# zprodev/zlib.es

Measured on AMD Instinct MI355X. Metric: GiB/s deflate+inflate round trip, 64 MiB buffers (uncompressed bytes / wall), bit-exact vs reference, higher is better.
Workload: dtype u8; 1 GPU; random64: 1 x 64 MiB xorshift buffer(s) per GPU (seed 12345+index), deflate then inflate, HBM-resident; bytes_per_buffer=67108864, compressed_bytes=67176156, parallelism=independent buffers, one per GPU

## Files before the change

### zlib.es_amd/csrc/zes_api.hip

```cpp
#include "../../include/zes.h"
#include "zes_kernels.h"
#include "zes_chain.h"

#include <algorithm>
#include <atomic>
#include <condition_variable>
#include <cstdio>
#include <cstddef>
#include <cstdlib>
#include <cstring>
#include <chrono>
#include <functional>
#include <future>
#include <initializer_list>
#include <deque>
#include <map>
#include <mutex>
#include <string>
#include <thread>
#include <vector>

extern "C" int zes_gen(uint8_t* out, uint64_t n, uint32_t kind, uint32_t seed);

namespace {
// ... 587 lines not shown

hipEvent_t take_event() {
  if (!g.event_pool.empty()) {
    hipEvent_t e = g.event_pool.back();
    g.event_pool.pop_back();
    return e;
  }
  hipEvent_t e = nullptr;
  (void)hipEventCreate(&e);
  return e;
}

struct Timed {
  hipEvent_t a = nullptr, b = nullptr;
  const char* name;
  hipStream_t st;
  explicit Timed(const char* n, hipStream_t stream = nullptr) : name(n), st(stream ? stream : g.stream) {
    if (g.profiling) {
      a = take_event();
      b = take_event();
      (void)hipEventRecord(a, st);
    }
  }
  ~Timed() {
    if (g.profiling) {
      (void)hipEventRecord(b, st);
      g.pending.push_back({name, {a, b}});
    }
    static const bool trace = getenv("ZES_TRACE_KERNELS") != nullptr;
    if (trace) {
      const hipError_t e = hipStreamSynchronize(g.stream);
      fprintf(stderr, "zes kernel done: %s (%s)\n", name, hipGetErrorName(e));
      fflush(stderr);
    }
  }
};

void collect_times() {
  if (!g.profiling) return;
  std::map<std::string, KTime> acc;
  std::vector<std::string> order;
  for (auto& p : g.pending) {
    float ms = 0;
    (void)hipEventSynchronize(p.second.second);
    (void)hipEventElapsedTime(&ms, p.second.first, p.second.second);
    if (!acc.count(p.first)) order.push_back(p.first);
    acc[p.first].ms += ms;
    acc[p.first].launches++;
    g.event_pool.push_back(p.second.first);
    g.event_pool.push_back(p.second.second);
  }
  g.pending.clear();
  g.last_times.clear();
  for (auto& e : g.carry) {
    auto it = acc.find(e.first);
    if (it != acc.end()) {
      e.second.ms += it->second.ms;
      e.second.launches += it->second.launches;
      acc.erase(it);
    }
    g.last_times.push_back(e);
  }
  g.carry.clear();
  for (auto& n : order)
    if (acc.count(n)) g.last_times.push_back({n, acc[n]});
}

void keep_times() {
  if (g.profiling) g.carry = g.last_times;
}

bool deflate_throws(uint64_t n) { return n == 0 || n == 1 || (n % ZES_BLK) == 1; }
uint64_t deflate_bound(uint64_t n) { return ((n < ZES_BLK / 2) ? (uint64_t)ZES_BLK : n * 2) + 6; }

using PhaseSetter = void (*)(unsigned long long*);
int phases_arm(PhaseSetter set, uint32_t nblk) {
  int rc = ensure(g.dbg, (size_t)nblk * 64);
  if (rc) return rc;
  HIPCHK(hipMemsetAsync(g.dbg.p, 0, (size_t)nblk * 64, g.stream));
  HIPCHK(hipStreamSynchronize(g.stream));
  set((unsigned long long*)g.dbg.p);
  return ZES_OK;
}
int phases_print(PhaseSetter set, uint32_t nblk, int ran, const char* fmt) {
  HIPCHK(hipStreamSynchronize(g.stream));
  set(nullptr);
  std::vector<unsigned long long> h((size_t)nblk * 8);
  HIPCHK(hipMemcpy(h.data(), g.dbg.p, h.size() * 8, hipMemcpyDeviceToHost));
  double acc[8] = {0};
  uint32_t n = 0;
  for (uint32_t i = 0; i < nblk; i++) {
    const unsigned long long* s = &h[(size_t)i * 8];
    if (!s[ran]) continue;
    n++;
    for (int k = 1; k < 8; k++) acc[k] += (double)(k <= ran ? s[k] - s[k - 1] : s[k]);
  }
  if (n) fprintf(stderr, fmt, n, acc[1] / n, acc[2] / n, acc[3] / n, acc[4] / n, acc[5] / n, acc[6] / n, acc[7] / n);
  return ZES_OK;
}

template <class F>
int launch_lz77(const uint8_t* d_in, uint32_t grid, bool use_index, bool heaviest_first, bool phases, F after_index, uint32_t* route = nullptr) {
  int rc;
  const ZesBuf* dbufs = (const ZesBuf*)g.bufs.p;
  ZesBlk* dblks = (ZesBlk*)g.blks.p;
  uint32_t* idx_a = (uint32_t*)g.idx_a.p;
  uint32_t* idx_b = (uint32_t*)g.idx_b.p;
  {
    Timed t("k_lz_sort");
    hipLaunchKernelGGL(k_lz_sort, dim3(grid), dim3(SORT_THREADS), 0, g.stream, d_in, dbufs, dblks, idx_a, idx_b, idx_a, (uint16_t*)g.sdelta.p,
                       ZES_SORT_MODE_FIRST | (use_index ? ZES_SORT_USE_INDEX : 0u));
  }
  auto note = [&](uint32_t* flag_to, uint32_t* word_to) -> int {
    HIPCHK(hipMemcpyAsync(flag_to, idx_a + ZES_BLK - 1, 4, hipMemcpyDeviceToHost, g.stream));
    if (word_to) HIPCHK(hipMemcpyAsync(word_to, idx_b + ZES_BLK - 1, 4, hipMemcpyDeviceToHost, g.stream));
    return ZES_OK;
  };
  if (route && (rc = note(&route[0], &route[3]))) return rc;
  if (use_index) {
    {
      Timed t("k_lz_index");
      hipLaunchKernelGGL(k_lz_index, dim3(grid), dim3(IDX_THREADS), 0, g.stream, d_in, dbufs, dblks, idx_a, idx_b, idx_a, (uint16_t*)g.sdelta.p);
    }
    if (route && (rc = note(&route[1], &route[4]))) return rc;
    {
      Timed t("k_lz_sort_redo");
      hipLaunchKernelGGL(k_lz_sort, dim3(grid), dim3(SORT_THREADS), 0, g.stream, d_in, dbufs, dblks, idx_a, idx_b, idx_a, (uint16_t*)g.sdelta.p,
                         ZES_SORT_MODE_REDO);
    }
    if (route && (rc = note(&route[2], nullptr))) return rc;
  }
  if ((rc = after_index())) return rc;
  {
    Timed t("k_lz_match");
    hipLaunchKernelGGL(k_lz_match, dim3(grid), dim3(MATCH_THREADS), 0, g.stream, d_in, dbufs, dblks, idx_a, idx_b, (uint32_t*)g.mlist.p);
  }
  if (phases && (rc = phases_arm(zes_lazy_set_dbg, grid))) return rc;
  {
    const uint32_t* order = nullptr;
    if (heaviest_first) {
      if ((rc = ensure(g.order, (size_t)grid * 4))) return rc;
      Timed t("k_lz_order");
      hipLaunchKernelGGL(k_lz_order, dim3(1), dim3(1024), 0, g.stream, (const uint32_t*)idx_a, grid, (uint32_t*)g.order.p);
      order = (const uint32_t*)g.order.p;
    }
    Timed t("k_lz_match_lazy");
    hipLaunchKernelGGL(k_lz_match_lazy, dim3(grid), dim3(MATCH_THREADS), 0, g.stream, d_in, dbufs, dblks, idx_a, (const uint32_t*)idx_a,
                       (const uint16_t*)g.sdelta.p, idx_b, (uint32_t*)g.tmask.p, (uint32_t*)g.mlist.p, order);
  }
  if (phases) {
    if ((rc = phases_print(zes_lazy_set_dbg, grid, 5,
                           "zes lazy match steps (avg cycles over %u blocks): stage %.0f tail %.0f window chains %.0f entry chains %.0f true chain (only unmerged blocks) %.0f | first wave, window chains: %.0f loop turns\n")))
      return rc;
    if ((rc = phases_arm(zes_parse_set_dbg, grid))) return rc;
  }
  {
    Timed t("k_lz_parse_small");
    hipLaunchKernelGGL(k_lz_parse_small, dim3(grid), dim3(PARSE_THREADS), 0, g.stream, d_in, dbufs, dblks, idx_b, idx_a, (uint32_t*)g.hists.p,
                       (const uint32_t*)g.tmask.p, (const uint32_t*)g.mlist.p);
  }
  {
    Timed t("k_lz_parse");
    hipLaunchKernelGGL(k_lz_parse, dim3(grid), dim3(PARSE_THREADS), 0, g.stream, d_in, dbufs, dblks, idx_b, idx_a, (uint32_t*)g.hists.p,
                       (const uint32_t*)g.tmask.p, (const uint32_t*)g.mlist.p);
  }
  return ZES_OK;
}

struct DeflateRange {
  uint64_t n_read = 0;
  uint32_t flags = 0;
  uint32_t start_bit = 0;
  bool defer = false;
  uint32_t adler = 1;
};

// ... 8 lines not shown
    out_len[i] = 0;
    if (deflate_throws(in_len[i])) {
      status[i] = ZES_E_CORRUPT;
      continue;
    }
    if (out_cap[i] < deflate_bound(in_len[i])) {
      status[i] = ZES_E_NOSPACE;
      out_len[i] = deflate_bound(in_len[i]);
      continue;
    }
    if ((out_off[i] & 15u) || (((uintptr_t)d_out) & 15u)) {
      status[i] = ZES_E_ARG;
      continue;
    }
    status[i] = ZES_OK;
    ZesBuf b;
    b.in_off = in_off[i];
    b.n = in_len[i];
    b.out_off = out_off[i];
    b.cap = out_cap[i];
    b.first_blk = (uint32_t)nblk_total;
    b.nblk = (uint32_t)((in_len[i] + ZES_BLK - 1) / ZES_BLK);
    b.n_read = one ? std::max(one->n_read, in_len[i]) : in_len[i];
    b.flags = one ? one->flags : 0u;
    b.start_bit = one ? one->start_bit : 0u;
    nblk_total += b.nblk;
    hb.push_back(b);
    live.push_back(i);
  }
  if (hb.empty()) return ZES_OK;
  if (nblk_total >= (1ull << 31)) return ZES_E_ARG;
  const uint32_t nbuf = (uint32_t)hb.size(), nblk = (uint32_t)nblk_total;
  int rc;
  if ((rc = ensure(g.bufs, sizeof(ZesBuf) * nbuf))) return rc;
  if ((rc = ensure(g.blks, sizeof(ZesBlk) * nblk))) return rc;
  if ((rc = ensure(g.idx_a, (size_t)nblk * ZES_BLK * 4))) return rc;
  if ((rc = ensure(g.idx_b, (size_t)nblk * ZES_BLK * 4))) return rc;
  if ((rc = ensure(g.sdelta, (size_t)nblk * ZES_BLK * 2 + 64))) return rc;
  if ((rc = ensure(g.tmask, (size_t)nblk * ZES_TMASK_WORDS * 4))) return rc;
  if ((rc = ensure(g.mlist, (size_t)nblk * ZES_MLIST_WORDS * 4))) return rc;
  if ((rc = ensure(g.hists, (size_t)nblk * 320 * 4))) return rc;
  if ((rc = ensure(g.codes, (size_t)nblk * 320 * 4))) return rc;
  if ((rc = ensure(g.hdrs, (size_t)nblk * ZES_HDR_WORDS * 4))) return rc;
  if ((rc = ensure(g.adler, (size_t)nbuf * 16))) return rc;
  if ((rc = ensure(g.res, sizeof(ZesRes) * nbuf))) return rc;
  ZesBuf* dbufs = (ZesBuf*)g.bufs.p;
  ZesBlk* dblks = (ZesBlk*)g.blks.p;
  unsigned long long* adler = (unsigned long long*)g.adler.p;
  if (nbuf > 1) {
    if (nbuf <= DEFLATE_TABLE_BUFS) {
      memcpy(g.pinned->def.table, hb.data(), sizeof(ZesBuf) * nbuf);
      HIPCHK(hipMemcpyAsync(g.bufs.p, g.pinned->def.table, sizeof(ZesBuf) * nbuf, hipMemcpyHostToDevice, g.stream));
    } else {
      HIPCHK(hipMemcpy(g.bufs.p, hb.data(), sizeof(ZesBuf) * nbuf, hipMemcpyHostToDevice));
    }
  }
  {
    Timed t("k_make_blks");
    const uint32_t nthr = std::max(nblk, 2u * nbuf);
    hipLaunchKernelGGL(k_make_blks, dim3((nthr + 255) / 256), dim3(256), 0, g.stream, hb[0], nbuf, dbufs, dblks, nblk, adler);
  }
  {
    HIPCHK(hipEventRecord(g.ev_a0, g.stream));
    HIPCHK(hipStreamWaitEvent(g.s_adler, g.ev_a0, 0));
    Timed t("k_adler", g.s_adler);
    if (nbuf == 1) {
      const uint32_t nch = (uint32_t)((hb[0].n + ADLER_CHUNK - 1) / ADLER_CHUNK);
      hipLaunchKernelGGL(k_adler, dim3(nch), dim3(ADLER_THREADS), 0, g.s_adler, d_in, hb[0].in_off, hb[0].n, adler);
    } else {
      hipLaunchKernelGGL(k_adler_blocks, dim3(nblk), dim3(ADLER_THREADS), 0, g.s_adler, d_in, dbufs, dblks, adler);
    }
  }
  HIPCHK(hipEventRecord(g.ev_a1, g.s_adler));
  const bool sort_dbg = getenv("ZES_DEBUG_PHASES") != nullptr;
  if (sort_dbg && (rc = phases_arm(zes_sort_set_dbg, nblk))) return rc;
  static const bool use_index = getenv("ZES_NO_INDEX") == nullptr;
  rc = launch_lz77(d_in, nblk, use_index, nbuf > 1 && nblk > 256, sort_dbg, [&]() -> int {
    if (!sort_dbg) return ZES_OK;
    return phases_print(zes_sort_set_dbg, nblk, 7,
                        "zes sort steps (avg cycles over %u blocks): zero %.0f count %.0f flags %.0f level 2 + compact %.0f stage %.0f three passes %.0f sd/inv %.0f\n");
  });
  if (rc) return rc;
  if (sort_dbg) {
    if ((rc = phases_print(zes_parse_set_dbg, nblk, 7, "zes parse steps (avg cycles over %u blocks): A %.0f B %.0f C %.0f D1 %.0f D2 %.0f D3 %.0f out %.0f\n"))) return rc;
    if ((rc = phases_arm(zes_huff_set_dbg, nblk))) return rc;
  }
  ZesRes* res_direct = (nbuf <= DEFLATE_DIRECT_BUFS && g.pinned_dev) ? g.pinned_dev->def.res : nullptr;
  {
    Timed t("k_huff");
    hipLaunchKernelGGL(k_huff, dim3(nblk), dim3(HUFF_THREADS_HOST), 0, g.stream, dblks, (const uint32_t*)g.hists.p,
                       (uint32_t*)g.codes.p, (uint32_t*)g.hdrs.p);
  }
  if (sort_dbg && (rc = phases_print(zes_huff_set_dbg, nblk, 7,
                                     "zes huff steps (avg cycles over %u blocks): rank sorts %.0f both alphabets' levels %.0f codes %.0f run-length coding %.0f its code %.0f header bits %.0f totals+out %.0f\n")))
    return rc;
  {
    HIPCHK(hipStreamWaitEvent(g.stream, g.ev_a1, 0));
    Timed t("k_layout");
    hipLaunchKernelGGL(k_layout, dim3(nbuf), dim3(256), 0, g.stream, d_out, dbufs, dblks, adler, res_direct ? res_direct : (ZesRes*)g.res.p);
  }
  if (sort_dbg && (rc = phases_arm(zes_emit_set_dbg, nblk))) return rc;
  {
    Timed t("k_emit");
    hipLaunchKernelGGL(k_emit, dim3(nblk), dim3(EMIT_THREADS), 0, g.stream, d_out, dbufs, dblks, (uint32_t*)g.idx_a.p,
                       (const uint32_t*)g.codes.p, (const uint32_t*)g.hdrs.p);
  }
  if (sort_dbg && (rc = phases_print(zes_emit_set_dbg, nblk, 1,
                                     "zes emit steps (avg cycles over %u blocks, first wave): whole %.0f = header copy %.0f build %.0f scan %.0f stage %.0f flush %.0f\n")))
    return rc;
  HIPCHK(hipGetLastError());
  ZesRes* r = g.pinned->def.res;
  if (nbuf > DEFLATE_DIRECT_BUFS) {
    if (nbuf > g.res_more_n) {
      if (g.res_more) HIPCHK(hipHostFree(g.res_more));
      g.res_more = nullptr;
      g.res_more_n = 0;
      HIPCHK(hipHostMalloc((void**)&g.res_more, sizeof(ZesRes) * nbuf * 2, hipHostMallocDefault));
      g.res_more_n = (size_t)nbuf * 2;
    }
    r = g.res_more;
  }
  if (!res_direct) HIPCHK(hipMemcpyAsync(r, g.res.p, sizeof(ZesRes) * nbuf, hipMemcpyDeviceToHost, g.stream));
  if (one && one->defer) return ZES_OK;
  HIPCHK(hipStreamSynchronize(g.stream));
  collect_times();
  for (uint32_t k = 0; k < nbuf; k++) {
    out_len[live[k]] = r[k].out_len;
    status[live[k]] = r[k].status;
  }
  if (one) one->adler = r[0].aux;
  return ZES_OK;
}

int deflate_one(const uint8_t* d_in, uint64_t in_off, uint64_t n, uint8_t* d_out, uint64_t out_off, uint64_t cap, uint64_t* out_len,
                DeflateRange* range = nullptr) {
  int32_t st = 0;
  const int rc = deflate_batch_core(d_in, &in_off, &n, d_out, &out_off, &cap, out_len, &st, 1, range);
  return rc ? rc : st;
}

int read_res(ZesRes* out) {
  HIPCHK(hipMemcpyAsync(&g.pinned->res1, g.res.p, sizeof(ZesRes), hipMemcpyDeviceToHost, g.stream));
  HIPCHK(hipStreamSynchronize(g.stream));
  *out = g.pinned->res1;
  return ZES_OK;
}

struct InfJob {
  uint64_t in_off, c, out_off, cap;
  uint64_t out_len;
  int status;
  int tier;
  uint32_t start0 = 16, hist = 0;
  bool partial = false, final_seen = false;
  uint64_t end_bit = 0;
  int btype0 = -1;
  bool want_end = false;
};

ZesInfBuf inf_buf(const InfJob& j) {
  ZesInfBuf b;
  memset(&b, 0, sizeof b);
  b.in_off = j.in_off;
  b.c = j.c;
  b.out_off = j.out_off;
  b.cap = j.cap;
  return b;
// ... 4913 lines not shown
```

### zlib.es_amd/csrc/zes_deflate.hip

```cpp
#include "zes_common.h"
#include "zes_kernels.h"

__device__ static inline uint32_t lds_ld32u(const uint8_t* s, uint32_t off) {
  const uint32_t* w = reinterpret_cast<const uint32_t*>(s);
  uint32_t i = off >> 2;
  uint32_t lo = w[i], hi = w[i + 1];
  return __builtin_amdgcn_alignbyte(hi, lo, off & 3u);
}

__device__ static inline void stage_block(uint8_t* s, const uint8_t* g, uint32_t bytes, uint32_t padded) {
  const uint32_t tid = threadIdx.x, nth = blockDim.x;
  const uint32_t mis = (uint32_t)((uintptr_t)g & 15u);
  if (mis == 0) {
    const uint4* g4 = reinterpret_cast<const uint4*>(g);
    uint4* s4 = reinterpret_cast<uint4*>(s);
    const uint32_t full = bytes >> 4;
    for (uint32_t i = tid; i < full; i += nth) s4[i] = g4[i];
    for (uint32_t i = (full << 4) + tid; i < padded; i += nth) s[i] = i < bytes ? g[i] : (uint8_t)0;
  } else {
    for (uint32_t i = tid; i < padded; i += nth) s[i] = i < bytes ? g[i] : (uint8_t)0;
  }
}

__device__ unsigned long long* g_sort_dbg = nullptr;
// ... 1646 lines not shown
              mo[base + lane] = LAZY_EVAL_LIT;
              atomicOr(&S.v1[(base + lane) >> 5], 1u << ((base + lane) & 31u));
            }
            p += nrun;
            continue;
          }
          if (++nev > budget3) {
            if (lane == 0) S.abort3 = 1u;
            break;
          }
          const uint32_t iv = (uint32_t)__builtin_amdgcn_readlane((int)ciw, (int)po);
          m = lazy_wave_eval(S, iv, sd, p, T, avail);
          if (lane == 0) mo[p] = m;
          if ((m & ZES_TOK_MATCH) && zes_tok_len(m) == ZES_MAXMATCH) {
            const uint32_t pj = p + ZES_MAXMATCH * (lane + 1u);
            const bool inr = pj < tbase && pj + ZES_MAXMATCH + 3u <= T && pj + ZES_MAXMATCH <= avail;
            const uint32_t ivj = inv[inr ? pj : 0u];
            const bool has = inr && ivj != ZES_INV_NONE;
            const uint32_t dj = sd[has ? (ivj & 0x1FFFFu) : 0u];
            const uint32_t qj = has ? pj - dj : 0u, pp = has ? pj : 0u;
            bool full = has;
            for (uint32_t wv = 0; wv < 32u && __ballot(full); wv += 4u) {
              uint64_t x = 0;
#pragma unroll
              for (uint32_t t = 0; t < 4u; t++) x |= lz_ld64(S.in, qj + 8u * (wv + t)) ^ lz_ld64(S.in, pp + 8u * (wv + t));
              full = full && x == 0ull;
            }
            full = full && ((lz_ld32(S.in, qj + 256u) ^ lz_ld32(S.in, pp + 256u)) & 0xffffu) == 0u;
            const uint64_t okm = __ballot(full);
            const uint32_t nk = (~okm) ? (uint32_t)__builtin_ctzll(~okm) : 64u;
            if (lane < nk) {
              mo[pj] = ZES_TOK_MATCH | ((ZES_MAXMATCH - 3u) << 16) | (dj - 1u);
              atomicOr(&S.v1[pj >> 5], 1u << (pj & 31u));
            }
            p += ZES_MAXMATCH * nk;
          }
        }
      }
      p += (m & ZES_TOK_MATCH) ? zes_tok_len(m) : 1u;
    }
    if (lane < 2u && cnt + lane < T && cnt + lane >= p) atomicOr(&S.v1[(cnt + lane) >> 5], 1u << ((cnt + lane) & 31u));
  }
  if (walk3) {
    __syncthreads();
    if (S.abort3) {
      probe = false;
      if (tid == 0) S.route |= ZES_ROUTE_ABORT3;
      __syncthreads();
      continue;
    }
    for (uint32_t i = tid; i < ZES_BLK / 32; i += MATCH_THREADS) tm[4u + i] = S.v1[i];
    __syncthreads();
    if (tid == 0) tm[0] = 1u;
  }
  break;
  }
  if (tid == 0) tm[1] = S.route;
  LSTAMP(5);
}

__device__ unsigned long long* g_parse_dbg = nullptr;
void zes_parse_set_dbg(unsigned long long* p) { (void)hipMemcpyToSymbol(HIP_SYMBOL(g_parse_dbg), &p, sizeof p); }
#define PSTAMP(i)                                                                                          \
  do {                                                                                                     \
    if (g_parse_dbg && threadIdx.x == 0) g_parse_dbg[(size_t)blockIdx.x * 8 + (i)] = (unsigned long long)clock64(); \
  } while (0)
#define PARSE_CHUNKS (ZES_BLK / 64)
#define PARSE_REGION 128
#define PARSE_NOENTRY 0xFFu
#define PARSE_BATCH 8u
template <bool SMALL>
struct ParseSmemT;
template <>
struct ParseSmemT<false> {
  union {
    uint8_t xmap[PARSE_CHUNKS][64];
    struct {
      unsigned long long mask[PARSE_CHUNKS];
      uint32_t cpre[PARSE_CHUNKS];
    } d;
  } u;
  uint16_t rtab[PARSE_THREADS / 64][5 * 64];
  uint8_t centry[PARSE_CHUNKS];
  uint8_t cplain[PARSE_CHUNKS];
  uint32_t rentry[PARSE_THREADS / 64 + 1];
  uint32_t wsum[PARSE_THREADS / 64];
  uint32_t lh[288];
  uint32_t dh[32];
};
template <>
struct ParseSmemT<true> {
  struct {
    struct {
      unsigned long long mask[PARSE_CHUNKS];
      uint32_t cpre[PARSE_CHUNKS];
    } d;
  } u;
  uint32_t srt[ZES_MLIST_WORDS];
  uint8_t acc[ZES_MLIST_WORDS];
  uint32_t mstart[ZES_BLK / 32];
  uint8_t cplain[PARSE_CHUNKS];
  uint32_t wsum[PARSE_THREADS / 64];
  uint32_t lh[288];
  uint32_t dh[32];
};

#define PARSE_ARRIVE8(a)                                                                                              \
  asm volatile("" : "+v"(a[0]), "+v"(a[1]), "+v"(a[2]), "+v"(a[3]), "+v"(a[4]), "+v"(a[5]), "+v"(a[6]), "+v"(a[7]))
static_assert(PARSE_BATCH == 8u, "PARSE_ARRIVE8 names eight registers");

__device__ static uint32_t parse_follow(const uint32_t* mi, uint32_t T, uint32_t chunk, uint32_t e) {
  uint32_t cur = e;
  while (cur < 64u) {
    const uint32_t p = chunk * 64u + cur;
    const uint32_t m = p < T ? mi[p] : 0u;
    cur += (m & ZES_TOK_MATCH) ? zes_tok_len(m) : 1u;
  }
  return cur - 64u;
}

#define PARSE_ARRIVE4(a) asm volatile("" : "+v"(a[0]), "+v"(a[1]), "+v"(a[2]), "+v"(a[3]))
template <bool SMALL>
__device__ __forceinline__ static void parse_body(ParseSmemT<SMALL>& S, const uint8_t* __restrict__ d_in, const ZesBuf* __restrict__ bufs,
                                                  ZesBlk* __restrict__ blks, const uint32_t* __restrict__ match_in,
                                                  uint32_t* __restrict__ tok_out, uint32_t* __restrict__ hists,
                                                  const uint32_t* __restrict__ tmask_all, const uint32_t* __restrict__ mlist_all) {
  const uint32_t g = blockIdx.x, tid = threadIdx.x, lane = tid & 63u, wave = tid >> 6;
  const ZesBlk bk = blks[g];
  const ZesBuf bf = bufs[bk.buf];
  const uint32_t T = bk.len;
  const uint8_t* src = d_in + bf.in_off + (uint64_t)bk.blk * ZES_BLK;
  const uint32_t* mi = match_in + (uint64_t)g * ZES_BLK;
  uint32_t* to = tok_out + (uint64_t)g * ZES_BLK;
  const uint32_t nchunks = (T + 63u) >> 6;
  const uint32_t nregions = (nchunks + PARSE_REGION - 1) / PARSE_REGION;
  const uint32_t* tmk = tmask_all + (uint64_t)g * ZES_TMASK_WORDS;
  const uint32_t* ml = mlist_all + (uint64_t)g * ZES_MLIST_WORDS;
  const uint32_t nml = ml[0];
  const bool lazyblk = nml == 0xFFFFFFFFu;
  const bool havemask = lazyblk && tmk[0] == 1u;
  const bool fewmatches = !lazyblk && nml <= ZES_MLIST_CAP;
  if (SMALL != (havemask || fewmatches)) return;
  for (uint32_t i = tid; i < 288; i += PARSE_THREADS) S.lh[i] = 0;
  if (tid < 32) S.dh[tid] = 0;
  if constexpr (!SMALL)
    for (uint32_t i = tid; i < PARSE_CHUNKS; i += PARSE_THREADS) S.centry[i] = PARSE_NOENTRY;
  PSTAMP(0);
  const uint32_t c_lo = wave * PARSE_REGION, c_hi = min(nchunks, c_lo + PARSE_REGION);
  if (havemask) {
    const unsigned long long* t64 = reinterpret_cast<const unsigned long long*>(tmk + 4);
    for (uint32_t c = tid; c < PARSE_CHUNKS; c += PARSE_THREADS) {
      S.u.d.mask[c] = c < nchunks ? t64[c] : 0ull;
      S.cplain[c] = 0;
    }
    __syncthreads();
  } else if (fewmatches) {
    if constexpr (SMALL) {
    uint16_t* wpre = reinterpret_cast<uint16_t*>(S.u.d.cpre);
    for (uint32_t c = tid; c < PARSE_CHUNKS; c += PARSE_THREADS) {
      const uint32_t lo = c * 64u;
      S.u.d.mask[c] = lo + 64u <= T ? ~0ull : (lo < T ? ((1ull << (T - lo)) - 1ull) : 0ull);
      S.cplain[c] = 1;
    }
    for (uint32_t i = tid; i < ZES_BLK / 32; i += PARSE_THREADS) S.mstart[i] = 0;
    __syncthreads();
    for (uint32_t i = tid; i < nml; i += PARSE_THREADS) {
      const uint32_t pe = ml[1u + i] & 0x1FFFFu;
      atomicOr(&S.mstart[pe >> 5], 1u << (pe & 31u));
    }
    __syncthreads();
    {
      static_assert(ZES_BLK / 32 == 4 * PARSE_THREADS, "four bitmap words per thread");
      uint32_t c4[4], sum = 0;
#pragma unroll
      for (uint32_t k = 0; k < 4; k++) {
        c4[k] = (uint32_t)__popc(S.mstart[4u * tid + k]);
        sum += c4[k];
      }
      uint32_t incl = sum;
#pragma unroll
      for (int dlt = 1; dlt < 64; dlt <<= 1) {
        const uint32_t t = __shfl_up(incl, dlt);
        if ((int)lane >= dlt) incl += t;
      }
      if (lane == 63) S.wsum[wave] = incl;
      __syncthreads();
      uint32_t run = incl - sum;
      for (uint32_t w = 0; w < wave; w++) run += S.wsum[w];
#pragma unroll
      for (uint32_t k = 0; k < 4; k++) {
        wpre[4u * tid + k] = (uint16_t)run;
        run += c4[k];
      }
    }
    __syncthreads();
    for (uint32_t i = tid; i < nml; i += PARSE_THREADS) {
      const uint32_t e = ml[1u + i], pe = e & 0x1FFFFu;
      const uint32_t r = (uint32_t)wpre[pe >> 5] + (uint32_t)__popc(S.mstart[pe >> 5] & ((1u << (pe & 31u)) - 1u));
      S.srt[r] = e;
    }
    __syncthreads();
    if (tid == 0) {
      uint32_t cur = 0;
      for (uint32_t i = 0; i < nml; i++) {
        const uint32_t e = S.srt[i], p = e & 0x1FFFFu, L = (e >> 17) + 3u;
        const bool take = p >= cur;
        S.acc[i] = take ? 1 : 0;
        cur = take ? p + L : cur;
      }
    }
    __syncthreads();
    for (uint32_t i = tid; i < nml; i += PARSE_THREADS) {
      const uint32_t e = S.srt[i], p = e & 0x1FFFFu, L = (e >> 17) + 3u;
      if (S.acc[i]) {
        S.cplain[p >> 6] = 0;
        for (uint32_t q = p + 1u; q < p + L;) {
          const uint32_t w = q >> 6, b0 = q & 63u, nb = min(64u - b0, p + L - q);
          const unsigned long long bits = (nb >= 64u ? ~0ull : ((1ull << nb) - 1ull)) << b0;
          atomicAnd(&S.u.d.mask[w], ~bits);
          q += nb;
        }
      } else {
        atomicAnd(&S.mstart[p >> 5], ~(1u << (p & 31u)));
      }
    }
    __syncthreads();
    }
  } else if constexpr (!SMALL) {
  for (uint32_t cb = c_lo; cb < c_hi; cb += PARSE_BATCH) {
    uint32_t mw[PARSE_BATCH];
#pragma unroll
    for (uint32_t k = 0; k < PARSE_BATCH; k++) {
      const uint32_t p = (cb + k) * 64u + lane;
      mw[k] = mi[min(p, T - 1u)];
    }
    PARSE_ARRIVE8(mw);
#pragma unroll
    for (uint32_t k = 0; k < PARSE_BATCH; k++) {
      const uint32_t c = cb + k;
      if (c >= c_hi) break;
      const uint32_t m = (c * 64u + lane < T) ? mw[k] : 0u;
      const bool plain = __ballot(m & ZES_TOK_MATCH) == 0ull;
      uint32_t v = lane + ((m & ZES_TOK_MATCH) ? zes_tok_len(m) : 1u);
      if (!plain) {
#pragma unroll
        for (int r = 0; r < 6; r++) {
          const uint32_t nv = __shfl(v, (int)(v & 63u));
          if (v < 64u) v = nv;
        }
      }
      S.u.xmap[c][lane] = plain ? (uint8_t)0 : (uint8_t)min(v - 64u, 255u);
      if (lane == 0) S.cplain[c] = plain ? 1 : 0;
    }
  }
  __syncthreads();

  PSTAMP(1);
  if (wave < nregions) {
    const uint32_t nch = c_hi - c_lo;
    uint32_t E1 = lane, E2 = 64u + lane, E3 = 128u + lane, E4 = 192u + lane, E5 = 256u + lane;
    for (int k = (int)nch - 1; k >= 0; k--) {
      const uint32_t c = c_lo + (uint32_t)k;
      uint32_t E0;
      if (S.cplain[c]) {
        E0 = (uint32_t)__builtin_amdgcn_readfirstlane((int)E1);
      } else {
        uint32_t ov = S.u.xmap[c][lane];
        if (ov == 255u) ov = parse_follow(mi, T, c, lane);
        const uint32_t d = ov >> 6, sl = ov & 63u;
        const uint32_t a1 = __shfl(E1, (int)sl), a2 = __shfl(E2, (int)sl), a3 = __shfl(E3, (int)sl), a4 = __shfl(E4, (int)sl),
                       a5 = __shfl(E5, (int)sl);
        E0 = d == 0 ? a1 : d == 1 ? a2 : d == 2 ? a3 : d == 3 ? a4 : a5;
      }
      E5 = E4;
      E4 = E3;
      E3 = E2;
      E2 = E1;
      E1 = E0;
    }
    S.rtab[wave][lane] = (uint16_t)E1;
    S.rtab[wave][64 + lane] = (uint16_t)E2;
    S.rtab[wave][128 + lane] = (uint16_t)E3;
    S.rtab[wave][192 + lane] = (uint16_t)E4;
    S.rtab[wave][256 + lane] = (uint16_t)E5;
  }
  __syncthreads();

  PSTAMP(2);
  if (tid == 0) {
    uint32_t e = 0;
    for (uint32_t r = 0; r < nregions; r++) {
      S.rentry[r] = e;
      e = S.rtab[r][e];
    }
  }
  __syncthreads();
  if (wave < nregions && lane == 0) {
    uint32_t cur = S.rentry[wave];
    const uint32_t lim = (c_hi - c_lo) * 64u;
    while (cur < lim) {
      const uint32_t c = c_lo + (cur >> 6), e = cur & 63u;
      S.centry[c] = (uint8_t)e;
      uint32_t ov = S.u.xmap[c][e];
      if (ov == 255u) ov = parse_follow(mi, T, c, e);
      cur = ((cur >> 6) + 1u) * 64u + ov;
    }
  }
  __syncthreads();

  PSTAMP(3);
  for (uint32_t cb = c_lo; cb < c_hi; cb += 64u) {
    const uint32_t c = cb + lane;
    const bool have = c < c_hi;
    const uint32_t cc = min(c, PARSE_CHUNKS - 1u);
    const uint32_t e = have ? (uint32_t)S.centry[cc] : PARSE_NOENTRY;
    const bool plain = S.cplain[cc] != 0;
    const uint32_t left = (have && cc * 64u < T) ? min(64u, T - cc * 64u) : 0u;
    unsigned long long mk = 0ull;
    if (e != PARSE_NOENTRY && plain)
      mk = (~0ull << e) & (left >= 64u ? ~0ull : ((1ull << left) - 1ull));
    uint32_t cur = (e != PARSE_NOENTRY && !plain) ? e : 64u;
    while (__ballot(cur < left)) {
      const bool act = cur < left;
      const uint32_t m = mi[act ? cc * 64u + cur : 0u];
      mk |= act ? (1ull << cur) : 0ull;
      cur += act ? ((m & ZES_TOK_MATCH) ? zes_tok_len(m) : 1u) : 0u;
    }
    if (have) S.u.d.mask[c] = mk;
  }
  __syncthreads();

  PSTAMP(4);
  }
  unsigned long long mymask[2] = {0ull, 0ull};
  uint32_t cnt2[2];
#pragma unroll
  for (int k = 0; k < 2; k++) {
    const uint32_t c = tid * 2 + k;
    mymask[k] = c < nchunks ? S.u.d.mask[c] : 0ull;
    cnt2[k] = (uint32_t)__popcll(mymask[k]);
  }
  const uint32_t mysum = cnt2[0] + cnt2[1];
  uint32_t incl = mysum;
#pragma unroll
  for (int dlt = 1; dlt < 64; dlt <<= 1) {
    const uint32_t t = __shfl_up(incl, dlt);
    if ((int)lane >= dlt) incl += t;
  }
  if (lane == 63) S.wsum[wave] = incl;
  __syncthreads();
  uint32_t wbase = 0, total = 0;
#pragma unroll
  for (uint32_t w = 0; w < PARSE_THREADS / 64; w++) {
    const uint32_t sm = S.wsum[w];
    if (w < wave) wbase += sm;
    total += sm;
  }
  const uint32_t ex = wbase + incl - mysum;
  if (tid * 2 < PARSE_CHUNKS) S.u.d.cpre[tid * 2] = ex;
  if (tid * 2 + 1 < PARSE_CHUNKS) S.u.d.cpre[tid * 2 + 1] = ex + cnt2[0];
  __syncthreads();

  PSTAMP(5);
  constexpr uint32_t DB = SMALL ? 4u : PARSE_BATCH;
  for (uint32_t cb = c_lo; cb < c_hi; cb += DB) {
    uint32_t mw[DB], by[DB];
    unsigned long long mks[DB];
    bool ism[DB];
#pragma unroll
    for (uint32_t k = 0; k < DB; k++) {
      const uint32_t c = cb + k;
      mks[k] = c < c_hi ? S.u.d.mask[c] : 0ull;
      const bool vis = (mks[k] >> lane) & 1ull;
      const uint32_t p = c * 64u + lane;
      by[k] = src[vis ? p : min(lane, T - 1u)];
      bool want = vis && !S.cplain[min(c, PARSE_CHUNKS - 1u)];
      if constexpr (SMALL) {
        const uint32_t pw = min(p, ZES_BLK - 1u);
        if (fewmatches) want = want && ((S.mstart[pw >> 5] >> (pw & 31u)) & 1u);
      }
      ism[k] = want;
      mw[k] = mi[want ? p : lane];
    }
    if constexpr (SMALL) {
      PARSE_ARRIVE4(by);
      PARSE_ARRIVE4(mw);
    } else {
      PARSE_ARRIVE8(by);
      PARSE_ARRIVE8(mw);
    }
#pragma unroll
    for (uint32_t k = 0; k < DB; k++) {
      const uint32_t c = cb + k;
      const unsigned long long mk = mks[k];
      if ((mk >> lane) & 1ull) {
        const uint32_t m = ism[k] ? mw[k] : 0u;
        const uint32_t rank = (uint32_t)__popcll(mk & zes_lanemask_lt());
        uint32_t tv;
        if (m & ZES_TOK_MATCH) {
          tv = m;
          atomicAdd(&S.lh[257u + zes_len_code(zes_tok_len(m))], 1u);
          atomicAdd(&S.dh[zes_dist_code(zes_tok_dist(m))], 1u);
        } else {
          tv = by[k];
          atomicAdd(&S.lh[tv], 1u);
        }
        to[S.u.d.cpre[c] + rank] = tv;
      }
    }
  }
  __syncthreads();
  PSTAMP(6);
  if (tid == 0) {
    S.lh[256] = 1;
    blks[g].ntok = total;
  }
  __syncthreads();
  uint32_t* hg = hists + (uint64_t)g * 320;
  for (uint32_t i = tid; i < 288; i += PARSE_THREADS) hg[i] = S.lh[i];
  if (tid < 32) hg[288 + tid] = S.dh[tid];
  PSTAMP(7);
}

__global__ __launch_bounds__(PARSE_THREADS) void k_lz_parse(const uint8_t* __restrict__ d_in, const ZesBuf* __restrict__ bufs,
                                                            ZesBlk* __restrict__ blks, const uint32_t* __restrict__ match_in,
                                                            uint32_t* __restrict__ tok_out, uint32_t* __restrict__ hists,
                                                            const uint32_t* __restrict__ tmask_all, const uint32_t* __restrict__ mlist_all) {
  __shared__ __align__(16) ParseSmemT<false> S;
  parse_body<false>(S, d_in, bufs, blks, match_in, tok_out, hists, tmask_all, mlist_all);
}
__global__ __launch_bounds__(PARSE_THREADS, 8) void k_lz_parse_small(const uint8_t* __restrict__ d_in, const ZesBuf* __restrict__ bufs,
                                                                     ZesBlk* __restrict__ blks, const uint32_t* __restrict__ match_in,
                                                                     uint32_t* __restrict__ tok_out, uint32_t* __restrict__ hists,
                                                                     const uint32_t* __restrict__ tmask_all,
                                                                     const uint32_t* __restrict__ mlist_all) {
  __shared__ __align__(16) ParseSmemT<true> S;
  parse_body<true>(S, d_in, bufs, blks, match_in, tok_out, hists, tmask_all, mlist_all);
}

__device__ unsigned long long* g_huff_dbg = nullptr;
void zes_huff_set_dbg(unsigned long long* p) { (void)hipMemcpyToSymbol(HIP_SYMBOL(g_huff_dbg), &p, sizeof p); }
#define USTAMP(i)                                                                                        \
  do {                                                                                                   \
    if (g_huff_dbg && threadIdx.x == 0) g_huff_dbg[(size_t)blockIdx.x * 8 + (i)] = (unsigned long long)clock64(); \
  } while (0)
#define HUFF_THREADS 384
#define HUFF_WAVES (HUFF_THREADS / 64)
#define PM_MAXN 320
static_assert(HUFF_THREADS == HUFF_THREADS_HOST && HUFF_THREADS == PM_MAXN + 64, "the lit/len team and the distance wavefront");
struct HuffSmem {
  uint32_t hist[320];
  alignas(16) uint32_t key[320];
  uint32_t lw[320];
  uint16_t lsym[320];
  alignas(8) uint32_t w[2][640];
  uint16_t leafpos[15][320];
  uint32_t pm_n[2];
  uint32_t a_k[2][16];
  uint32_t top[3];
  uint8_t lens[320];
  uint8_t clens[32];
  uint16_t codes[320];
  uint16_t ccodes[32];
  uint8_t rl_sym[320];
  uint8_t rl_val[320];
  uint32_t hdr[ZES_HDR_WORDS];
  uint32_t hdr_bits;
  uint32_t total_bits;
  uint32_t ccount[2][16], cfirst[2][16];
  uint16_t cwave[HUFF_WAVES][16];
  uint8_t cl[320];
  uint32_t wsum[HUFF_WAVES];
  unsigned long long starts[5];
};

struct PmTeam {
  uint32_t t, size, base;
};
template <bool kWave>
__device__ __forceinline__ static void pm_sync() {
  if (kWave) asm volatile("s_waitcnt lgkmcnt(0)" ::: "memory");
  else __syncthreads();
}

template <bool kWave>
__device__ static void pm_lengths(HuffSmem& S, const PmTeam T, uint32_t nsym, uint32_t L, uint8_t* lens, int stamp) {
  const uint32_t lane = threadIdx.x & 63u, b = T.base, a = b ? 1u : 0u;
  const uint32_t i = T.t < T.size ? T.t : PM_MAXN;
  const uint32_t key = (i < nsym ? S.hist[b + i] : 0u) - 1u;
  if (i < (b ? 32u : 288u)) S.key[b + i] = key;
  if (T.t == 0) S.pm_n[a] = 0;
  if (i < nsym) lens[i] = 0;
  pm_sync<kWave>();
  const bool used = key != ~0u;
  uint32_t rank = 0;
  if (used) {
    const uint32_t own = __builtin_amdgcn_readfirstlane(i & ~63u);
    const uint4* k4 = reinterpret_cast<const uint4*>(S.key + b);
    for (uint32_t q = 0; q < own >> 2; q++) {
      const uint4 k = k4[q];
      rank += (k.x <= key) + (k.y <= key) + (k.z <= key) + (k.w <= key);
    }
    for (uint32_t q = own >> 2, qe = min(own + 64u, (nsym + 3u) & ~3u) >> 2; q < qe; q++) {
      const uint4 k = k4[q];
// ... 891 lines not shown
```

### zlib.es_amd/csrc/zes_kernels.h

```cpp
#pragma once
#include "zes_common.h"

#define SORT_THREADS 1024
#define SORT_WAVES (SORT_THREADS / 64)
#ifndef MATCH_THREADS
#define MATCH_THREADS 1024
#endif
#define IDX_THREADS 1024
#define ZES_SORT_LAZY 0x80000000u
#define ZES_SORT_INDEX 0x40000000u
#define ZES_SORT_REDO 0x20000000u
#define ZES_INV_NONE 0xFFFFFFFFu
#define ZES_ROUTE_WORDS 9u
#define ZES_ROUTE_SORT_TWO 1u
#define ZES_ROUTE_SORT_DENSE 2u
#define ZES_ROUTE_IDX_MAXC 0x3FFFFu
#define ZES_ROUTE_IDX_GROUP 0x40000000u
#define ZES_ROUTE_IDX_HEAVY 0x80000000u
#define ZES_ROUTE_GUARDED 1u
#define ZES_ROUTE_PROBED 2u
#define ZES_ROUTE_PERIODIC 4u
#define ZES_ROUTE_ABORT3 8u
#define ZES_ROUTE_LATE_CLEAR 16u
#define ZES_ROUTE_WALK3 32u
// ... 200 lines not shown
  uint64_t src_off;
  uint64_t dst_off;
  uint32_t height, rowbytes;
  uint32_t bpp;
  uint32_t mode;
  uint32_t first_unit;
  uint32_t pad;
};
#define ZES_PNGW_BANDED 5u
#define ZES_PNGW_ADAPTIVE 6u
#define ZES_PNGW_RUN 16u
#define ZES_PNGW_THREADS 256u
struct ZesPngwRec {
  uint64_t src_off;
  uint64_t dst_off;
  uint64_t zlen;
  uint64_t adler_off;
  uint32_t flen;
  uint32_t width, height;
  uint32_t aux_off;
  uint32_t first_wg;
  uint32_t adler;
  uint16_t plte_len, trns_len;
  uint8_t depth, colour, stored, pad;
};
#define ZES_PNGW_NO_SLOT 0xFFFFFFFFFFFFFFFFull
#define ZES_PNGW_IDAT 65536u
#define ZES_PNGW_BLOCK 65535u
struct ZesCrcPut {
  uint64_t dst;
  uint32_t mul, add;
};

uint32_t zes_crc_shift(uint32_t s, uint64_t k);
uint32_t zes_crc_mul(uint32_t a, uint32_t b);
uint32_t zes_crc_host(const uint8_t* p, uint64_t n);
void zes_crc_tables(uint32_t* tab, uint32_t npow);

#ifdef __HIPCC__
__global__ void k_inf_first_bytes(const uint8_t*, const uint64_t*, uint8_t*, uint32_t);
__global__ void k_inf_scan(const uint8_t*, const ZesInfBuf*, uint32_t, unsigned long long*, uint32_t, uint32_t*, uint8_t*, uint32_t,
                           const uint8_t*);
__global__ void k_inf_set_table1(ZesInfBuf, ZesInfBuf, ZesInfBuf*, uint32_t*, uint32_t);
__global__ void k_inf_verify(const uint8_t*, const ZesInfBuf*, const unsigned long long*, uint32_t, uint32_t*, uint32_t*, uint32_t*, uint32_t, uint32_t*, uint32_t, uint32_t);
__global__ void k_inf_verify_long(const uint8_t*, const ZesInfBuf*, const unsigned long long*, uint32_t, uint32_t*, uint32_t*, uint32_t*, uint32_t, const uint32_t*, uint32_t);
__global__ void k_inf_ranksort(const ZesInfBuf*, const uint32_t*, const uint32_t*, uint32_t*, uint32_t);
__global__ void k_inf_decode(const uint8_t*, uint8_t*, const ZesInfBuf*, ZesRes*, uint64_t*);
__global__ void k_inf_stored_walk(const uint8_t*, uint64_t, uint64_t, uint64_t, ZesStoredBlk*, ZesRes*);
__global__ void k_inf_stored_copy(const uint8_t*, uint64_t, uint8_t*, uint64_t, const ZesStoredBlk*);
__global__ void k_inf_stored_find(const uint8_t*, uint64_t, uint32_t, uint32_t*, uint32_t*);
__global__ void k_inf_stored_rank(const uint8_t*, uint64_t, uint32_t, const uint32_t*, const uint32_t*, uint32_t, uint64_t, ZesStoredBlk*, ZesRes*);
__global__ void k_inf_cand_bucket(const uint32_t*, const uint32_t*, uint32_t, uint32_t, uint32_t*);
__global__ void k_inf_cand_compact(const uint32_t*, uint32_t*, uint32_t*);
__global__ void k_inf_seg_order(const ZesSegJob*, const uint32_t*, uint32_t*);
__global__ void k_inf_seg_scan(const uint8_t*, const ZesSegJob*, uint32_t, const uint32_t*, ZesSegRes*, uint32_t*, uint32_t*, uint32_t,
                               const uint32_t*, uint32_t*, const uint32_t*, uint64_t*);
__global__ void k_inf_seg_scan_short(const uint8_t*, const ZesSegJob*, uint32_t, const uint32_t*, ZesSegRes*, uint32_t*, uint32_t*, uint32_t,
                                     const uint32_t*, uint32_t*, const uint32_t*, uint64_t*);
__global__ void k_inf_seg_block_par(const uint8_t*, const ZesSegJob*, uint32_t, const uint32_t*, ZesSegRes*, uint32_t*, uint32_t*, uint32_t, uint32_t*,
                                    unsigned long long*, uint64_t, uint64_t, uint64_t*, unsigned long long*);
__global__ void k_inf_seg_chain(const ZesSegJob*, const ZesSegRes*, uint32_t*, uint64_t*, ZesRes*, uint32_t*);
__global__ void k_inf_seg_translate(uint8_t*, const ZesSegJob*, const ZesSegOut*, const uint32_t*, const ZesSegRes*, const uint32_t*, const uint64_t*,
                                    const uint8_t*, const uint32_t*, const uint64_t*, uint32_t*);
#define SEGWIN_GROUP 32u
__global__ void k_inf_seg_win_group(const uint32_t*, const uint32_t*, const ZesSegJob*, uint32_t*);
__global__ void k_inf_seg_win_top(const uint32_t*, const ZesSegJob*, uint8_t*, const uint8_t*, const ZesSegOut*);
__global__ void k_inf_seg_win_fin(const uint32_t*, const ZesSegJob*, const uint8_t*, uint8_t*);
__global__ void k_inf_seg_decode(const uint8_t*, uint64_t, uint64_t, uint8_t*, uint64_t, uint64_t, const uint32_t*, const ZesSegRes*,
                                 const uint32_t*, const uint64_t*, const uint8_t*, uint32_t*, uint32_t, uint32_t, uint32_t);
__global__ void k_inf_block_par(const uint8_t*, uint8_t*, const ZesInfBuf*, uint32_t, const uint32_t*, const uint32_t*, const uint32_t*,
                                ZesCandRes*, unsigned long long*, const uint32_t*, const uint32_t*, uint32_t*, ZesParMirror);
__global__ void k_inf_block_par2(const uint8_t*, uint8_t*, const ZesInfBuf*, uint32_t, const uint32_t*, const uint32_t*, const uint32_t*,
                                ZesCandRes*, unsigned long long*, const uint32_t*, const uint32_t*, uint32_t*, ZesParMirror);
__global__ void k_inf_move_slots(uint8_t*, const uint8_t*, const uint32_t*, const uint32_t*, uint32_t);
__global__ void k_inf_chain(const ZesInfBuf*, const uint32_t*, const uint32_t*, const ZesCandRes*, const uint32_t*, uint32_t*, ZesRes*, const uint32_t*, uint32_t, uint32_t*);
__global__ void k_inf_chain_range(const ZesInfBuf*, const uint32_t*, const uint32_t*, const ZesCandRes*, ZesRes*, unsigned long long*);
__global__ void k_inf_set_table_range(ZesInfBuf, ZesInfBuf, ZesInfBuf*, uint32_t*, uint32_t, const unsigned long long*, unsigned long long);
__global__ void k_inf_exact(const uint8_t*, uint64_t, uint64_t, uint8_t*, uint64_t, uint64_t, const uint64_t*, ZesRes*);
void zes_sort_set_dbg(unsigned long long*);
#ifdef WD_PROFILE
void zes_wd_set_dbg(unsigned long long*);
#endif
void zes_parse_set_dbg(unsigned long long*);
void zes_lazy_set_dbg(unsigned long long*);
void zes_huff_set_dbg(unsigned long long*);
void zes_emit_set_dbg(unsigned long long*);
__global__ void k_make_blks(ZesBuf, uint32_t, ZesBuf*, ZesBlk*, uint32_t, unsigned long long*);
__global__ void k_lz_sort(const uint8_t*, const ZesBuf*, const ZesBlk*, uint32_t*, uint32_t*, uint32_t*, uint16_t*, uint32_t);
__global__ void k_lz_index(const uint8_t*, const ZesBuf*, const ZesBlk*, uint32_t*, uint32_t*, uint32_t*, uint16_t*);
#define ZES_SORT_MODE_FIRST 0u
#define ZES_SORT_MODE_REDO 1u
#define ZES_SORT_USE_INDEX 256u
__global__ void k_lz_match_lazy(const uint8_t*, const ZesBuf*, const ZesBlk*, const uint32_t*, const uint32_t*, const uint16_t*, uint32_t*, uint32_t*, uint32_t*,
                                const uint32_t*);
__global__ void k_lz_order(const uint32_t*, uint32_t, uint32_t*);
__global__ void k_lz_match(const uint8_t*, const ZesBuf*, const ZesBlk*, const uint32_t*, uint32_t*, uint32_t*);
__global__ void k_lz_parse(const uint8_t*, const ZesBuf*, ZesBlk*, const uint32_t*, uint32_t*, uint32_t*, const uint32_t*, const uint32_t*);
__global__ void k_lz_parse_small(const uint8_t*, const ZesBuf*, ZesBlk*, const uint32_t*, uint32_t*, uint32_t*, const uint32_t*, const uint32_t*);
__global__ void k_huff(ZesBlk*, const uint32_t*, uint32_t*, uint32_t*);
__global__ void k_huff_lengths_only(const uint32_t*, uint32_t, uint32_t, uint8_t*);
__global__ void k_selftest_lds_order(unsigned long long*, uint32_t, uint32_t);
__global__ void k_adler(const uint8_t*, uint64_t, uint64_t, unsigned long long*);
__global__ void k_crc32(const uint8_t*, uint64_t, const uint32_t*, unsigned int*);
__global__ void k_crc32_seg(const uint8_t*, const ZesCrcSeg*, const uint2*, const uint32_t*, unsigned int*);
__global__ void k_gz_walk(const uint8_t*, uint64_t, ZesGzWalk*, ZesGzMember*, uint32_t);
__global__ void k_bgzf_mark(const uint8_t*, uint64_t, ZesBgzfMark*, ZesBgzfCand*, uint32_t);
__global__ void k_gz_gather(const uint8_t*, uint8_t*, const ZesGzSeg*);
__global__ void k_bgzf_pack(const uint8_t*, const uint8_t*, uint8_t*, const ZesBgzfRec*);
__global__ void k_zip_stage(const uint8_t*, uint8_t*, uint8_t*, const ZesZipRec*, ZesZipVerdict*);
__global__ void k_zip_pack(const uint8_t*, const uint8_t*, const uint8_t*, uint8_t*, const ZesZipPackRec*, uint32_t);
__global__ void k_png_walk(const uint8_t*, const ZesPngFile*, uint32_t, ZesPngHead*, ZesPngChunk*);
__global__ void k_png_unfilter(const uint8_t*, uint8_t*, const ZesPngJob*, uint32_t, uint32_t, uint32_t*);
__global__ void k_png_expand(const uint8_t*, const uint8_t*, uint8_t*, const ZesPngxJob*, uint32_t);
__global__ void k_png_filter(const uint8_t*, uint8_t*, const ZesPngwJob*, uint32_t);
__global__ void k_png_pack(const uint8_t*, const uint8_t*, const uint8_t*, uint8_t*, const ZesPngwRec*, uint32_t);
__global__ void k_crc32_put(const unsigned int*, const ZesCrcPut*, uint32_t, uint8_t*);
__global__ void k_adler_blocks(const uint8_t*, const ZesBuf*, const ZesBlk*, unsigned long long*);
__global__ void k_adler_seg(const uint8_t*, const ZesCrcSeg*, const uint2*, unsigned long long*);
__global__ void k_layout(uint8_t*, const ZesBuf*, ZesBlk*, const unsigned long long*, ZesRes*);
__global__ void k_emit(uint8_t*, const ZesBuf*, const ZesBlk*, const uint32_t*, const uint32_t*, const uint32_t*);
__global__ void k_zero_u64(unsigned long long*, uint32_t);
__global__ void k_bits_place(uint32_t*, uint64_t, const uint32_t*, uint64_t);
#endif
```

Before: 50.91 GiB/s.

## Parallelize match acceptance walk and restructure parse token output by word rows

Replaces the single-thread serial greedy acceptance walk over the sorted match list with a pointer-jumping (doubling) pass over next-match link tables stored where the masks will later live. Rewrites the token emission loop to load source bytes as 32-bit words and match tokens as uint4 per lane, with software prefetch of the next row batches and a fast path for all-literal rows. Adds per-route debug stamps and filtered phase printing. The aim is to remove serial latency and byte-granular loads in the parse kernel, at the cost of more syncs per doubling step and more complex alignment handling.

```diff
diff --git a/zlib.es_amd/csrc/zes_api.hip b/zlib.es_amd/csrc/zes_api.hip
--- a/zlib.es_amd/csrc/zes_api.hip
+++ b/zlib.es_amd/csrc/zes_api.hip
@@ -693,7 +693,7 @@
   set((unsigned long long*)g.dbg.p);
   return ZES_OK;
 }
-int phases_print(PhaseSetter set, uint32_t nblk, int ran, const char* fmt) {
+int phases_print(PhaseSetter set, uint32_t nblk, int ran, const char* fmt, unsigned long long lo7 = 0, unsigned long long hi7 = ~0ull) {
   HIPCHK(hipStreamSynchronize(g.stream));
   set(nullptr);
   std::vector<unsigned long long> h((size_t)nblk * 8);
@@ -702,7 +702,7 @@
   uint32_t n = 0;
   for (uint32_t i = 0; i < nblk; i++) {
     const unsigned long long* s = &h[(size_t)i * 8];
-    if (!s[ran]) continue;
+    if (!s[ran] || s[7] < lo7 || s[7] > hi7) continue;
     n++;
     for (int k = 1; k < 8; k++) acc[k] += (double)(k <= ran ? s[k] - s[k - 1] : s[k]);
   }
@@ -877,7 +877,17 @@
   });
   if (rc) return rc;
   if (sort_dbg) {
-    if ((rc = phases_print(zes_parse_set_dbg, nblk, 7, "zes parse steps (avg cycles over %u blocks): A %.0f B %.0f C %.0f D1 %.0f D2 %.0f D3 %.0f out %.0f\n"))) return rc;
+    if ((rc = phases_print(zes_parse_set_dbg, nblk, 7, "zes parse steps (avg cycles over %u blocks): A %.0f B %.0f C %.0f D1 %.0f D2 %.0f D3 %.0f out %.0f\n",
+                           PARSE_DBG_MASK + 1)))
+      return rc;
+    if ((rc = phases_print(zes_parse_set_dbg, nblk, 6,
+                           "zes parse steps, list route (avg cycles over %u blocks): bitmap + rank %.0f acceptance walk %.0f chain mask cleared %.0f D2 %.0f D3 %.0f out %.0f\n",
+                           PARSE_DBG_LIST, PARSE_DBG_LIST)))
+      return rc;
+    if ((rc = phases_print(zes_parse_set_dbg, nblk, 6,
+                           "zes parse steps, mask route (avg cycles over %u blocks): mask read %.0f (no walk) %.0f (no clearing) %.0f D2 %.0f D3 %.0f out %.0f\n",
+                           PARSE_DBG_MASK, PARSE_DBG_MASK)))
+      return rc;
     if ((rc = phases_arm(zes_huff_set_dbg, nblk))) return rc;
   }
   ZesRes* res_direct = (nbuf <= DEFLATE_DIRECT_BUFS && g.pinned_dev) ? g.pinned_dev->def.res : nullptr;
diff --git a/zlib.es_amd/csrc/zes_deflate.hip b/zlib.es_amd/csrc/zes_deflate.hip
--- a/zlib.es_amd/csrc/zes_deflate.hip
+++ b/zlib.es_amd/csrc/zes_deflate.hip
@@ -1752,7 +1752,7 @@
   } u;
   uint16_t rtab[PARSE_THREADS / 64][5 * 64];
   uint8_t centry[PARSE_CHUNKS];
-  uint8_t cplain[PARSE_CHUNKS];
+  alignas(4) uint8_t cplain[PARSE_CHUNKS];
   uint32_t rentry[PARSE_THREADS / 64 + 1];
   uint32_t wsum[PARSE_THREADS / 64];
   uint32_t lh[288];
@@ -1769,7 +1769,7 @@
   uint32_t srt[ZES_MLIST_WORDS];
   uint8_t acc[ZES_MLIST_WORDS];
   uint32_t mstart[ZES_BLK / 32];
-  uint8_t cplain[PARSE_CHUNKS];
+  alignas(4) uint8_t cplain[PARSE_CHUNKS];
   uint32_t wsum[PARSE_THREADS / 64];
   uint32_t lh[288];
   uint32_t dh[32];
@@ -1789,7 +1789,8 @@
   return cur - 64u;
 }
 
-#define PARSE_ARRIVE4(a) asm volatile("" : "+v"(a[0]), "+v"(a[1]), "+v"(a[2]), "+v"(a[3]))
+#define PARSE_DR 2u
+#define PARSE_PF 2u
 template <bool SMALL>
 __device__ __forceinline__ static void parse_body(ParseSmemT<SMALL>& S, const uint8_t* __restrict__ d_in, const ZesBuf* __restrict__ bufs,
                                                   ZesBlk* __restrict__ blks, const uint32_t* __restrict__ match_in,
@@ -1824,14 +1825,13 @@
       S.cplain[c] = 0;
     }
     __syncthreads();
+    PSTAMP(1);
+    PSTAMP(2);
+    PSTAMP(3);
   } else if (fewmatches) {
     if constexpr (SMALL) {
     uint16_t* wpre = reinterpret_cast<uint16_t*>(S.u.d.cpre);
-    for (uint32_t c = tid; c < PARSE_CHUNKS; c += PARSE_THREADS) {
-      const uint32_t lo = c * 64u;
-      S.u.d.mask[c] = lo + 64u <= T ? ~0ull : (lo < T ? ((1ull << (T - lo)) - 1ull) : 0ull);
-      S.cplain[c] = 1;
-    }
+    for (uint32_t c = tid; c < PARSE_CHUNKS; c += PARSE_THREADS) S.cplain[c] = 1;
     for (uint32_t i = tid; i < ZES_BLK / 32; i += PARSE_THREADS) S.mstart[i] = 0;
     __syncthreads();
     for (uint32_t i = tid; i < nml; i += PARSE_THREADS) {
@@ -1870,14 +1870,37 @@
       S.srt[r] = e;
     }
     __syncthreads();
-    if (tid == 0) {
+    PSTAMP(1);
+    {
+      static_assert(2u * ZES_MLIST_WORDS * sizeof(uint16_t) <= sizeof(S.u.d.mask), "two link tables where the masks will stand");
+      uint16_t* jmp = reinterpret_cast<uint16_t*>(S.u.d.mask);
+      for (uint32_t i = tid; i <= nml; i += PARSE_THREADS) {
+        uint32_t nx = nml;
+        if (i < nml) {
+          const uint32_t e = S.srt[i], end = min((e & 0x1FFFFu) + (e >> 17) + 3u, ZES_BLK - 1u);
+          nx = (uint32_t)wpre[end >> 5] + (uint32_t)__popc(S.mstart[end >> 5] & ((1u << (end & 31u)) - 1u));
+        }
+        jmp[i] = (uint16_t)nx;
+        S.acc[i] = i == 0u ? 1 : 0;
+      }
       uint32_t cur = 0;
-      for (uint32_t i = 0; i < nml; i++) {
-        const uint32_t e = S.srt[i], p = e & 0x1FFFFu, L = (e >> 17) + 3u;
-        const bool take = p >= cur;
-        S.acc[i] = take ? 1 : 0;
-        cur = take ? p + L : cur;
-      }
+      for (uint32_t span = 1; span < nml; span <<= 1) {
+        __syncthreads();
+        const uint16_t* ja = jmp + cur * ZES_MLIST_WORDS;
+        uint16_t* jb = jmp + (cur ^ 1u) * ZES_MLIST_WORDS;
+        for (uint32_t i = tid; i <= nml; i += PARSE_THREADS) {
+          const uint32_t j = ja[i];
+          if (S.acc[i]) S.acc[j] = 1;
+          jb[i] = ja[j];
+        }
+        cur ^= 1u;
+      }
+    }
+    __syncthreads();
+    PSTAMP(2);
+    for (uint32_t c = tid; c < PARSE_CHUNKS; c += PARSE_THREADS) {
+      const uint32_t lo = c * 64u;
+      S.u.d.mask[c] = lo + 64u <= T ? ~0ull : (lo < T ? ((1ull << (T - lo)) - 1ull) : 0ull);
     }
     __syncthreads();
     for (uint32_t i = tid; i < nml; i += PARSE_THREADS) {
@@ -1895,6 +1918,7 @@
       }
     }
     __syncthreads();
+    PSTAMP(3);
     }
   } else if constexpr (!SMALL) {
   for (uint32_t cb = c_lo; cb < c_hi; cb += PARSE_BATCH) {
@@ -2026,61 +2050,97 @@
     if (w < wave) wbase += sm;
     total += sm;
   }
+  total = (uint32_t)__builtin_amdgcn_readfirstlane((int)total);
   const uint32_t ex = wbase + incl - mysum;
   if (tid * 2 < PARSE_CHUNKS) S.u.d.cpre[tid * 2] = ex;
   if (tid * 2 + 1 < PARSE_CHUNKS) S.u.d.cpre[tid * 2 + 1] = ex + cnt2[0];
   __syncthreads();
 
-  PSTAMP(5);
-  constexpr uint32_t DB = SMALL ? 4u : PARSE_BATCH;
-  for (uint32_t cb = c_lo; cb < c_hi; cb += DB) {
-    uint32_t mw[DB], by[DB];
-    unsigned long long mks[DB];
-    bool ism[DB];
-#pragma unroll
-    for (uint32_t k = 0; k < DB; k++) {
-      const uint32_t c = cb + k;
-      mks[k] = c < c_hi ? S.u.d.mask[c] : 0ull;
-      const bool vis = (mks[k] >> lane) & 1ull;
-      const uint32_t p = c * 64u + lane;
-      by[k] = src[vis ? p : min(lane, T - 1u)];
-      bool want = vis && !S.cplain[min(c, PARSE_CHUNKS - 1u)];
-      if constexpr (SMALL) {
-        const uint32_t pw = min(p, ZES_BLK - 1u);
-        if (fewmatches) want = want && ((S.mstart[pw >> 5] >> (pw & 31u)) & 1u);
-      }
-      ism[k] = want;
-      mw[k] = mi[want ? p : lane];
-    }
-    if constexpr (SMALL) {
-      PARSE_ARRIVE4(by);
-      PARSE_ARRIVE4(mw);
-    } else {
-      PARSE_ARRIVE8(by);
-      PARSE_ARRIVE8(mw);
-    }
-#pragma unroll
-    for (uint32_t k = 0; k < DB; k++) {
-      const uint32_t c = cb + k;
-      const unsigned long long mk = mks[k];
-      if ((mk >> lane) & 1ull) {
-        const uint32_t m = ism[k] ? mw[k] : 0u;
-        const uint32_t rank = (uint32_t)__popcll(mk & zes_lanemask_lt());
-        uint32_t tv;
-        if (m & ZES_TOK_MATCH) {
-          tv = m;
-          atomicAdd(&S.lh[257u + zes_len_code(zes_tok_len(m))], 1u);
-          atomicAdd(&S.dh[zes_dist_code(zes_tok_dist(m))], 1u);
-        } else {
-          tv = by[k];
-          atomicAdd(&S.lh[tv], 1u);
-        }
-        to[S.u.d.cpre[c] + rank] = tv;
-      }
-    }
-  }
-  __syncthreads();
-  PSTAMP(6);
+  constexpr int PD = SMALL ? 4 : 5;
+  PSTAMP(PD);
+  static_assert((PARSE_REGION / 4u) % PARSE_DR == 0u, "a region is a whole number of row batches");
+  const uint32_t mis = (uint32_t)((uintptr_t)src & 3u);
+  const uint32_t* srcw = reinterpret_cast<const uint32_t*>(src - mis);
+  const uint32_t lastw = (T + mis - 1u) >> 2;
+  const uint32_t woff = mis ? 1u : 0u;
+  const uint4* mi4 = reinterpret_cast<const uint4*>(mi);
+  const uint32_t r_lo = wave * (PARSE_REGION / 4u), r_hi = c_hi > c_lo ? (c_hi + 3u) >> 2 : r_lo;
+  const uint32_t sub = lane >> 4, nsh = (lane & 15u) * 4u;
+  uint32_t nw[PARSE_PF][PARSE_DR];
+#pragma unroll
+  for (uint32_t i = 0; i < PARSE_PF; i++)
+#pragma unroll
+    for (uint32_t k = 0; k < PARSE_DR; k++) nw[i][k] = srcw[min((r_lo + i * PARSE_DR + k) * 64u + lane + woff, lastw)];
+  uint32_t carry = srcw[min(r_lo * 64u, lastw)];
+  for (uint32_t rb0 = r_lo; rb0 < r_hi; rb0 += PARSE_PF * PARSE_DR) {
+#pragma unroll
+  for (uint32_t pf = 0; pf < PARSE_PF; pf++) {
+    const uint32_t rb = rb0 + pf * PARSE_DR;
+    if (rb >= r_hi) break;
+    uint32_t w[PARSE_DR], nb[PARSE_DR];
+    uint4 mw[PARSE_DR];
+#pragma unroll
+    for (uint32_t k = 0; k < PARSE_DR; k++) {
+      const uint32_t R = rb + k, c = R * 4u + sub;
+      w[k] = nw[pf][k];
+      const unsigned long long mk = c < c_hi ? S.u.d.mask[c] : 0ull;
+      const uint32_t nib = (uint32_t)(mk >> nsh) & 15u;
+      uint32_t wn = S.cplain[c] ? 0u : nib;
+      if constexpr (SMALL)
+        if (fewmatches) wn &= S.mstart[R * 8u + (lane >> 3)] >> ((lane & 7u) * 4u);
+      nb[k] = nib | (wn << 4);
+      mw[k] = make_uint4(0u, 0u, 0u, 0u);
+      if (wn) mw[k] = mi4[R * 64u + lane];
+    }
+#pragma unroll
+    for (uint32_t k = 0; k < PARSE_DR; k++) nw[pf][k] = srcw[min((rb + PARSE_PF * PARSE_DR + k) * 64u + lane + woff, lastw)];
+#pragma unroll
+    for (uint32_t k = 0; k < PARSE_DR; k++) {
+      const uint32_t R = rb + k, nib = nb[k] & 15u, wn = nb[k] >> 4;
+      if (__ballot(nib != 0u) == 0ull) continue;
+      uint32_t b = w[k];
+      if (mis) {
+        uint32_t lo = __shfl_up(b, 1);
+        const uint32_t below = k ? (uint32_t)__builtin_amdgcn_readlane((int)w[k ? k - 1u : 0u], 63) : carry;
+        if (lane == 0) lo = below;
+        b = __builtin_amdgcn_alignbyte(b, lo, mis);
+      }
+      const bool lits = *reinterpret_cast<const uint32_t*>(&S.cplain[R * 4u]) == 0x01010101u && __ballot(nib == 15u) == ~0ull;
+      if (lits) {
+        atomicAdd(&S.lh[b & 255u], 1u);
+        atomicAdd(&S.lh[(b >> 8) & 255u], 1u);
+        atomicAdd(&S.lh[(b >> 16) & 255u], 1u);
+        atomicAdd(&S.lh[b >> 24], 1u);
+        const uint32_t tb = S.u.d.cpre[R * 4u];
+#pragma unroll
+        for (uint32_t q = 0; q < 4; q++)
+          to[tb + q * 64u + lane] = ((uint32_t)__shfl((int)b, (int)(q * 16u + (lane >> 2))) >> (8u * (lane & 3u))) & 255u;
+      } else {
+        uint32_t at = S.u.d.cpre[R * 4u + sub] + (uint32_t)__popcll(S.u.d.mask[R * 4u + sub] & ((1ull << nsh) - 1ull));
+        const uint32_t mv[4] = {mw[k].x, mw[k].y, mw[k].z, mw[k].w};
+#pragma unroll
+        for (uint32_t j = 0; j < 4; j++) {
+          if ((nib >> j) & 1u) {
+            const uint32_t m = ((wn >> j) & 1u) ? mv[j] : 0u;
+            uint32_t tv;
+            if (m & ZES_TOK_MATCH) {
+              tv = m;
+              atomicAdd(&S.lh[257u + zes_len_code(zes_tok_len(m))], 1u);
+              atomicAdd(&S.dh[zes_dist_code(zes_tok_dist(m))], 1u);
+            } else {
+              tv = (b >> (8u * j)) & 255u;
+              atomicAdd(&S.lh[tv], 1u);
+            }
+            to[at++] = tv;
+          }
+        }
+      }
+    }
+    if (mis) carry = (uint32_t)__builtin_amdgcn_readlane((int)w[PARSE_DR - 1u], 63);
+  }
+  }
+  __syncthreads();
+  PSTAMP(PD + 1);
   if (tid == 0) {
     S.lh[256] = 1;
     blks[g].ntok = total;
@@ -2089,7 +2149,9 @@
   uint32_t* hg = hists + (uint64_t)g * 320;
   for (uint32_t i = tid; i < 288; i += PARSE_THREADS) hg[i] = S.lh[i];
   if (tid < 32) hg[288 + tid] = S.dh[tid];
-  PSTAMP(7);
+  PSTAMP(PD + 2);
+  if constexpr (SMALL)
+    if (g_parse_dbg && tid == 0) g_parse_dbg[(size_t)g * 8 + 7] = fewmatches ? PARSE_DBG_LIST : PARSE_DBG_MASK;
 }
 
 __global__ __launch_bounds__(PARSE_THREADS) void k_lz_parse(const uint8_t* __restrict__ d_in, const ZesBuf* __restrict__ bufs,
diff --git a/zlib.es_amd/csrc/zes_kernels.h b/zlib.es_amd/csrc/zes_kernels.h
--- a/zlib.es_amd/csrc/zes_kernels.h
+++ b/zlib.es_amd/csrc/zes_kernels.h
@@ -306,6 +306,8 @@
 void zes_wd_set_dbg(unsigned long long*);
 #endif
 void zes_parse_set_dbg(unsigned long long*);
+#define PARSE_DBG_LIST 1ull
+#define PARSE_DBG_MASK 2ull
 void zes_lazy_set_dbg(unsigned long long*);
 void zes_huff_set_dbg(unsigned long long*);
 void zes_emit_set_dbg(unsigned long long*);
```

Result: no change. 51.02 GiB/s, median of 2 (+0.2%).
